# davmacario/MDI-LLM

Measured on AMD Instinct MI355X. Metric: llama3_8b_pipeline_decode_tok_per_s, higher is better.
Workload: dtype bf16; 1 GPU; model=Meta-Llama-3-8B-Instruct, global_batch=1, seq_len=128, max_seq_len=2048, parallelism=pp1, samples_in_flight=1, group_size=1, backend=hip

## Files before the change

mdi_llm_amd/ops/hip/decode_kernels.hip:

```cpp

#include <cstdlib>
#include <type_traits>
#include <hip/hip_runtime.h>
#include <hip/hip_bf16.h>

#include "decode_kernels.h"

#define DEVINL __device__ __forceinline__

using bf16 = __hip_bfloat16;

DEVINL float b2f(bf16 v) { return __bfloat162float(v); }
DEVINL bf16 f2b(float v) { return __float2bfloat16(v); }

struct bf16x8 {
  bf16 v[8];
};

DEVINL bf16x8 load8(const bf16* p) {
  bf16x8 r;
  *reinterpret_cast<int4*>(r.v) = *reinterpret_cast<const int4*>(p);
  return r;
}

using i32x4_t = __attribute__((ext_vector_type(4))) int;

DEVINL bf16x8 load8_nt(const bf16* p) {
  bf16x8 r;
  *reinterpret_cast<i32x4_t*>(r.v) =
      __builtin_nontemporal_load(reinterpret_cast<const i32x4_t*>(p));
  return r;
}

DEVINL i32x4_t load16_nt_u8(const unsigned char* p) {
  return __builtin_nontemporal_load(reinterpret_cast<const i32x4_t*>(p));
}

using f32x4 = __attribute__((__vector_size__(16))) float;
using bf16x8_t = __attribute__((ext_vector_type(8))) __bf16;

DEVINL float wave_reduce_max(float v) {
#pragma unroll
  for (int off = 32; off > 0; off >>= 1)
    v = fmaxf(v, __shfl_xor(v, off, 64));
  return v;
}

using u8kv = unsigned char;
typedef float v2fkv __attribute__((ext_vector_type(2)));

DEVINL u8kv f32_to_fp8(float f) {
  const int packed = __builtin_amdgcn_cvt_pk_fp8_f32(f, 0.f, 0, false);
  return (u8kv)(packed & 0xFF);
}

DEVINL float fp8_to_f32(u8kv v) {
  return __builtin_amdgcn_cvt_f32_fp8((int)v, 0);
}

DEVINL bf16x8_t fp8x8_to_bf16(const u8kv* p, float scl) {
  const int lo = *reinterpret_cast<const int*>(p);
  const int hi = *reinterpret_cast<const int*>(p + 4);
  const v2fkv a = __builtin_amdgcn_cvt_pk_f32_fp8(lo, false);
  const v2fkv b = __builtin_amdgcn_cvt_pk_f32_fp8(lo, true);
  const v2fkv c = __builtin_amdgcn_cvt_pk_f32_fp8(hi, false);
  const v2fkv d = __builtin_amdgcn_cvt_pk_f32_fp8(hi, true);
  bf16x8_t r;
  r[0] = (__bf16)(a.x * scl);
  r[1] = (__bf16)(a.y * scl);
  r[2] = (__bf16)(b.x * scl);
  r[3] = (__bf16)(b.y * scl);
  r[4] = (__bf16)(c.x * scl);
  r[5] = (__bf16)(c.y * scl);
  r[6] = (__bf16)(d.x * scl);
  r[7] = (__bf16)(d.y * scl);
  return r;
}

DEVINL void fp8x8_fma(float* o, float pw, const u8kv* p, float scl) {
  const int lo = *reinterpret_cast<const int*>(p);
  const int hi = *reinterpret_cast<const int*>(p + 4);
  const v2fkv a = __builtin_amdgcn_cvt_pk_f32_fp8(lo, false);
  const v2fkv b = __builtin_amdgcn_cvt_pk_f32_fp8(lo, true);
  const v2fkv c = __builtin_amdgcn_cvt_pk_f32_fp8(hi, false);
  const v2fkv d = __builtin_amdgcn_cvt_pk_f32_fp8(hi, true);
  const float ps = pw * scl;
  o[0] += ps * a.x;
  o[1] += ps * a.y;
  o[2] += ps * b.x;
  o[3] += ps * b.y;
  o[4] += ps * c.x;
  o[5] += ps * c.y;
  o[6] += ps * d.x;
  o[7] += ps * d.y;
}

DEVINL void lds_fmax_u(unsigned* addr, float v) {
  atomicMax(addr, __float_as_uint(v));
}

DEVINL float wave_reduce_sum(float v) {
#pragma unroll
  for (int off = 32; off > 0; off >>= 1) v += __shfl_xor(v, off, 64);
  return v;
}

__global__ void rmsnorm_kernel(bf16* __restrict__ out,
                               const bf16* __restrict__ x,
                               const bf16* __restrict__ w, int n, float eps) {
  __shared__ float red[4];
  out += (size_t)blockIdx.y * n;
  x += (size_t)blockIdx.y * n;
  const int tid = threadIdx.x;
  float acc = 0.f;
  for (int i = tid * 8; i < n; i += blockDim.x * 8) {
    bf16x8 v = load8(x + i);
#pragma unroll
    for (int j = 0; j < 8; ++j) {
      float f = b2f(v.v[j]);
      acc += f * f;
    }
  }
  acc = wave_reduce_sum(acc);
  if ((tid & 63) == 0) red[tid >> 6] = acc;
  __syncthreads();
  float total = red[0] + red[1] + red[2] + red[3];
  float scale = rsqrtf(total / n + eps);
  for (int i = tid * 8; i < n; i += blockDim.x * 8) {
    bf16x8 v = load8(x + i);
    bf16x8 g = load8(w + i);
    bf16x8 o;
#pragma unroll
    for (int j = 0; j < 8; ++j)
      o.v[j] = f2b(b2f(v.v[j]) * scale * b2f(g.v[j]));
    *reinterpret_cast<int4*>(out + i) = *reinterpret_cast<const int4*>(o.v);
  }
}

__global__ void layernorm_kernel(bf16* __restrict__ out,
                                 const bf16* __restrict__ x,
                                 const bf16* __restrict__ w,
                                 const bf16* __restrict__ b, int n,
                                 float eps) {
  __shared__ float red[8];
  const int tid = threadIdx.x;
  float s = 0.f, s2 = 0.f;
  for (int i = tid * 8; i < n; i += blockDim.x * 8) {
    bf16x8 v = load8(x + i);
#pragma unroll
    for (int j = 0; j < 8; ++j) {
      float f = b2f(v.v[j]);
      s += f;
      s2 += f * f;
    }
  }
  s = wave_reduce_sum(s);
  s2 = wave_reduce_sum(s2);
  if ((tid & 63) == 0) {
    red[(tid >> 6) * 2] = s;
    red[(tid >> 6) * 2 + 1] = s2;
  }
  __syncthreads();
  float mean = (red[0] + red[2] + red[4] + red[6]) / n;
  float var = (red[1] + red[3] + red[5] + red[7]) / n - mean * mean;
  float inv = rsqrtf(var + eps);
  for (int i = tid * 8; i < n; i += blockDim.x * 8) {
    bf16x8 v = load8(x + i);
    bf16x8 g = load8(w + i);
    bf16x8 o;
    if (b != nullptr) {
      bf16x8 bb = load8(b + i);
#pragma unroll
      for (int j = 0; j < 8; ++j)
        o.v[j] = f2b((b2f(v.v[j]) - mean) * inv * b2f(g.v[j]) + b2f(bb.v[j]));
    } else {
#pragma unroll
      for (int j = 0; j < 8; ++j)
// ... 865 lines not shown
  }
}

__global__ void swiglu_mul_kernel(bf16* __restrict__ out,
                                  const bf16* __restrict__ g,
                                  const bf16* __restrict__ u,
                                  long long n, int gelu_gate) {
  const long long i0 = ((long long)blockIdx.x * blockDim.x + threadIdx.x) * 8;
  const long long stride = (long long)gridDim.x * blockDim.x * 8;
  for (long long i = i0; i < n; i += stride) {
    bf16x8 gv = load8(g + i);
    bf16x8 uv = load8(u + i);
    bf16x8 o;
#pragma unroll
    for (int j = 0; j < 8; ++j) {
      const float gf = b2f(gv.v[j]);
      const float act = gelu_gate ? gelu_tanh(gf)
                                  : gf / (1.f + __expf(-gf));
      o.v[j] = f2b(act * b2f(uv.v[j]));
    }
    *reinterpret_cast<int4*>(out + i) = *reinterpret_cast<const int4*>(o.v);
  }
}

__global__ void embed_kernel(bf16* __restrict__ out,
                             const bf16* __restrict__ wte,
                             const int* __restrict__ token, int n_embd,
                             float scale) {
  const int t = token[0];
  const bf16* row = wte + (size_t)t * n_embd;
  for (int i = (blockIdx.x * blockDim.x + threadIdx.x) * 8; i < n_embd;
       i += gridDim.x * blockDim.x * 8) {
    bf16x8 v = load8(row + i);
    if (scale != 1.f) {
#pragma unroll
      for (int j = 0; j < 8; ++j) v.v[j] = f2b(b2f(v.v[j]) * scale);
    }
    *reinterpret_cast<int4*>(out + i) = *reinterpret_cast<const int4*>(v.v);
  }
}

__global__ void rope_kv_append_kernel(
    bf16* __restrict__ qkv, bf16* __restrict__ kpool,
    bf16* __restrict__ vpool, const float* __restrict__ cos_t,
    const float* __restrict__ sin_t, const int* __restrict__ pos_p,
    const int* __restrict__ slot_p, int layer, int n_layers_pool,
    int n_kv_heads, int max_seq, int head_size, int rope_n_elem, int qpk) {
  const int g = blockIdx.x;
  const int pos = pos_p[0];
  const int slot = slot_p[0];
  const int tid = threadIdx.x;
  const int half = rope_n_elem >> 1;

  bf16* base = qkv + (size_t)g * (qpk + 2) * head_size;

  for (int idx = tid; idx < (qpk + 1) * half; idx += blockDim.x) {
    const int r = idx / half;
    const int d = idx % half;
    bf16* row = base + (size_t)r * head_size;
    float x1 = b2f(row[d]);
    float x2 = b2f(row[d + half]);
    float c1 = cos_t[(size_t)pos * rope_n_elem + d];
    float s1 = sin_t[(size_t)pos * rope_n_elem + d];
    float c2 = cos_t[(size_t)pos * rope_n_elem + d + half];
    float s2 = sin_t[(size_t)pos * rope_n_elem + d + half];
    row[d] = f2b(x1 * c1 - x2 * s1);
    row[d + half] = f2b(x2 * c2 + x1 * s2);
  }
  __syncthreads();

  const size_t cache_off =
      (((size_t)slot * n_layers_pool + layer) * n_kv_heads + g) *
          (size_t)max_seq * head_size +
      (size_t)pos * head_size;
  const bf16* krow = base + (size_t)qpk * head_size;
  const bf16* vrow = base + (size_t)(qpk + 1) * head_size;
  for (int d = tid; d < head_size; d += blockDim.x) {
    kpool[cache_off + d] = krow[d];
    vpool[cache_off + d] = vrow[d];
  }
}

#define ATTN_WAVES 4
#define ATTN_BLOCK_MAX_SEQ 4096

template <int HS>
DEVINL int q_swz(int row, int d) {
  int byte = (row * HS + d) * 2;
  byte ^= (row & 7) << 4;
  return byte >> 1;
}

DEVINL float rope_elem(const bf16* row, int d, int ne,
                       const float* __restrict__ cos_t,
                       const float* __restrict__ sin_t, int pos) {
  float x = b2f(row[d]);
  if (d >= ne) return x;
  const int half = ne >> 1;
  const float c = cos_t[(size_t)pos * ne + d];
  const float s = sin_t[(size_t)pos * ne + d];
  if (d < half) return x * c - b2f(row[d + half]) * s;
  return x * c + b2f(row[d - half]) * s;
}

template <int QPK, int HS, int BATCH, int KV8>
__global__ void attn_decode_block_kernel(
    bf16* __restrict__ out,
    const bf16* __restrict__ qkv,
    void* __restrict__ kpool_v, void* __restrict__ vpool_v,
    float* __restrict__ kscale, float* __restrict__ vscale,
    const float* __restrict__ cos_t, const float* __restrict__ sin_t,
    int rope_ne, const int* __restrict__ pos_p,
    const int* __restrict__ slot_p, int layer, int n_layers_pool,
    int n_kv_heads, int max_seq, float scale, int n_batch) {
  using kvt = std::conditional_t<KV8 != 0, u8kv, bf16>;
  kvt* kpool = reinterpret_cast<kvt*>(kpool_v);
  kvt* vpool = reinterpret_cast<kvt*>(vpool_v);
  constexpr int head_size = HS;
  static_assert(HS % 32 == 0 && HS * QPK >= 64, "unsupported attn geometry");
  constexpr int ODIM = HS * QPK / 64;

  __shared__ __attribute__((aligned(16))) bf16 q_lds[16 * HS];
  __shared__ __attribute__((aligned(16))) bf16 k_cur[HS];
  __shared__ float o_part[ATTN_WAVES][QPK][HS];
  __shared__ float ml_part[ATTN_WAVES][QPK][2];
  __shared__ unsigned kvmax[2];

  const int wave = threadIdx.x >> 6;
  const int lane = threadIdx.x & 63;
  const int b = BATCH ? (int)blockIdx.x / n_kv_heads : 0;
  const int g = BATCH ? (int)blockIdx.x % n_kv_heads : (int)blockIdx.x;
  if (b >= n_batch) return;

  const int S = pos_p[b] + 1;
  const int pos = S - 1;
  const int slot = slot_p[b];
  const int n_head_all = n_kv_heads * QPK;
  if (BATCH) {
    const int qkv_dim = n_kv_heads * (QPK + 2) * head_size;
    qkv += (size_t)b * qkv_dim;
    out += (size_t)b * n_head_all * head_size;
  }

  const size_t cache_base =
      (((size_t)slot * n_layers_pool + layer) * n_kv_heads + g) *
      (size_t)max_seq * head_size;
  const size_t scl_base =
      (((size_t)slot * n_layers_pool + layer) * n_kv_heads + g) *
      (size_t)max_seq;
  const bf16* krow_cur = qkv + ((size_t)g * (QPK + 2) + QPK) * head_size;
  const bf16* vrow_cur = krow_cur + head_size;
  if (KV8 && threadIdx.x < 2) kvmax[threadIdx.x] = 0;

  for (int i = threadIdx.x; i < (16 - QPK) * head_size / 8; i += 256)
    reinterpret_cast<bf16x8_t*>(q_lds + QPK * head_size)[i] = bf16x8_t{};
  for (int i = threadIdx.x; i < QPK * head_size; i += 256) {
    const int r = i / head_size;
    const int d = i % head_size;
    const bf16* qrow = qkv + ((size_t)g * (QPK + 2) + r) * head_size;
    q_lds[q_swz<HS>(r, d)] =
        f2b(rope_elem(qrow, d, rope_ne, cos_t, sin_t, pos));
  }
  for (int d = threadIdx.x; d < head_size; d += 256)
    k_cur[d] = f2b(rope_elem(krow_cur, d, rope_ne, cos_t, sin_t, pos));
  __syncthreads();

  if constexpr (KV8) {
    float lk = 0.f, lv = 0.f;
    for (int d = threadIdx.x; d < head_size; d += 256) {
      lk = fmaxf(lk, fabsf(b2f(k_cur[d])));
      lv = fmaxf(lv, fabsf(b2f(vrow_cur[d])));
    }
    lds_fmax_u(&kvmax[0], lk);
    lds_fmax_u(&kvmax[1], lv);
    __syncthreads();
    const float ks = fmaxf(__uint_as_float(kvmax[0]), 1e-12f) / 448.f;
    const float vs = fmaxf(__uint_as_float(kvmax[1]), 1e-12f) / 448.f;
    for (int d = threadIdx.x; d < head_size; d += 256) {
      kpool[cache_base + (size_t)pos * head_size + d] =
          f32_to_fp8(b2f(k_cur[d]) / ks);
      vpool[cache_base + (size_t)pos * head_size + d] =
          f32_to_fp8(b2f(vrow_cur[d]) / vs);
    }
    if (threadIdx.x == 0) {
      kscale[scl_base + pos] = ks;
      vscale[scl_base + pos] = vs;
    }
  } else {
    for (int d = threadIdx.x; d < head_size; d += 256) {
      kpool[cache_base + (size_t)pos * head_size + d] = k_cur[d];
      vpool[cache_base + (size_t)pos * head_size + d] = vrow_cur[d];
    }
  }

  const int qa = lane & 15;
  const int sub = lane >> 4;
  const int qb = lane % QPK;
  const int d0 = (lane / QPK) * ODIM;

  float m_st = -1e30f, l_st = 0.f;
  float o_acc[ODIM];
#pragma unroll
  for (int i = 0; i < ODIM; ++i) o_acc[i] = 0.f;

  const int n_tiles = (S + 15) / 16;
  for (int t = wave; t < n_tiles; t += ATTN_WAVES) {
    const int key0 = t * 16;

    f32x4 acc4 = {0.f, 0.f, 0.f, 0.f};
    const int arow = lane & 15;
    const int koff = (lane >> 4) * 8;
    const int akey = key0 + arow;
    const kvt* krow = kpool + cache_base + (size_t)akey * head_size;
    const bool row_valid = akey < S;
    const bool row_cur = akey == pos;
    float kscl = 1.f;
    if (KV8 && row_valid && !row_cur) kscl = kscale[scl_base + akey];
#pragma unroll
    for (int c = 0; c < HS / 32; ++c) {
      bf16x8_t af = {};
      if (row_cur)
        af = *reinterpret_cast<const bf16x8_t*>(&k_cur[c * 32 + koff]);
      else if (row_valid) {
        if constexpr (KV8)
          af = fp8x8_to_bf16(
              reinterpret_cast<const u8kv*>(krow) + c * 32 + koff, kscl);
        else
          af = *reinterpret_cast<const bf16x8_t*>(
              reinterpret_cast<const bf16*>(krow) + c * 32 + koff);
      }
      const bf16x8_t bq = *reinterpret_cast<const bf16x8_t*>(
          &q_lds[q_swz<HS>(arow, c * 32 + koff)]);
      acc4 = __builtin_amdgcn_mfma_f32_16x16x32_bf16(af, bq, acc4, 0, 0, 0);
    }
    float sc[4];
#pragma unroll
    for (int r = 0; r < 4; ++r) {
      const int key = key0 + sub * 4 + r;
      sc[r] = (key < S) ? acc4[r] * scale : -1e30f;
    }

    float tmax = fmaxf(fmaxf(sc[0], sc[1]), fmaxf(sc[2], sc[3]));
    tmax = fmaxf(tmax, __shfl_xor(tmax, 16, 64));
    tmax = fmaxf(tmax, __shfl_xor(tmax, 32, 64));
    const float m_new = fmaxf(m_st, tmax);
    const float alpha = __expf(m_st - m_new);
    m_st = m_new;
    float e[4];
    float psum = 0.f;
#pragma unroll
    for (int r = 0; r < 4; ++r) {
      const int key = key0 + sub * 4 + r;
      e[r] = (key < S) ? __expf(sc[r] - m_new) : 0.f;
      psum += e[r];
    }
    psum += __shfl_xor(psum, 16, 64);
    psum += __shfl_xor(psum, 32, 64);
    l_st = l_st * alpha + psum;

    const float alphaB = __shfl(alpha, qb, 64);
#pragma unroll
    for (int i = 0; i < ODIM; ++i) o_acc[i] *= alphaB;
#pragma unroll
    for (int s = 0; s < 16; ++s) {
      const float p = __shfl(e[s & 3], ((s >> 2) << 4) | qb, 64);
      const int skey = min(key0 + s, pos);
      const bool vcur = skey == pos;
      const bf16* vrow_b = vrow_cur + d0;
      const kvt* vrow_p = vpool + cache_base + (size_t)skey * head_size + d0;
      float vscl = 1.f;
      if (KV8 && !vcur) vscl = vscale[scl_base + skey];
      if constexpr (ODIM >= 8) {
#pragma unroll
        for (int i = 0; i < ODIM; i += 8) {
          if (!vcur) {
            if constexpr (KV8) {
              fp8x8_fma(&o_acc[i], p,
                        reinterpret_cast<const u8kv*>(vrow_p) + i, vscl);
              continue;
            }
          }
          bf16x8_t vv;
          if (vcur) {
            vv = *reinterpret_cast<const bf16x8_t*>(vrow_b + i);
          } else {
            vv = *reinterpret_cast<const bf16x8_t*>(
                reinterpret_cast<const bf16*>(vrow_p) + i);
          }
#pragma unroll
          for (int j = 0; j < 8; ++j) o_acc[i + j] += p * (float)vv[j];
        }
      } else {
#pragma unroll
        for (int j = 0; j < ODIM; ++j) {
          float v;
          if (vcur)
            v = b2f(vrow_b[j]);
          else if constexpr (KV8)
            v = fp8_to_f32(reinterpret_cast<const u8kv*>(vrow_p)[j]) * vscl;
          else
            v = b2f(reinterpret_cast<const bf16*>(vrow_p)[j]);
          o_acc[j] += p * v;
        }
      }
    }
  }

#pragma unroll
  for (int i = 0; i < ODIM; ++i) o_part[wave][qb][d0 + i] = o_acc[i];
  if (lane < QPK) {
    ml_part[wave][lane][0] = m_st;
    ml_part[wave][lane][1] = l_st;
  }
  __syncthreads();

  for (int i = threadIdx.x; i < QPK * head_size; i += 256) {
    const int h = i / head_size;
    const int d = i % head_size;
    float M = -1e30f;
#pragma unroll
    for (int w = 0; w < ATTN_WAVES; ++w)
      M = fmaxf(M, ml_part[w][h][0]);
    float den = 0.f, num = 0.f;
#pragma unroll
    for (int w = 0; w < ATTN_WAVES; ++w) {
      const float wgt = __expf(ml_part[w][h][0] - M);
      den += wgt * ml_part[w][h][1];
      num += wgt * o_part[w][h][d];
    }
    out[(size_t)(g * QPK + h) * head_size + d] = f2b(num / den);
  }
}

typedef __attribute__((address_space(1))) unsigned int gu32_t;

template <int QPK, int HS, int THROTTLE>
__global__ void attn_proj_kernel(
    bf16* __restrict__ out,
    const bf16* __restrict__ qkv,
    bf16* __restrict__ kpool, bf16* __restrict__ vpool,
    const float* __restrict__ cos_t, const float* __restrict__ sin_t,
    int rope_ne, const int* __restrict__ pos_p,
    const int* __restrict__ slot_p, int layer, int n_layers_pool,
    int n_kv_heads, int max_seq, float scale,
    const bf16* __restrict__ W,
    const bf16* __restrict__ bias,
    const bf16* __restrict__ res,
    unsigned int* __restrict__ gran,
    int M, int BR) {
  constexpr int head_size = HS;
  constexpr int ODIM = HS * QPK / 64;
  extern __shared__ __attribute__((aligned(16))) char smem[];

  const int K = n_kv_heads * QPK * head_size;
  const int tid = threadIdx.x;
  const int wave = tid >> 6;
  const int lane = tid & 63;
  const int S = pos_p[0] + 1;
  const int pos = S - 1;
  const int slot = slot_p[0];
  const unsigned tag = (unsigned)(slot * max_seq + S);
  gu32_t* g32 = (gu32_t*)gran;
  gu32_t* flags = g32 + K / 2;

  if ((int)blockIdx.x >= n_kv_heads) {
    const int pb = (int)blockIdx.x - n_kv_heads;
    const int PBe = (int)gridDim.x - n_kv_heads;
    bf16* wlds = reinterpret_cast<bf16*>(smem);
    int* vflag = reinterpret_cast<int*>(smem + (size_t)BR * K * 2);
    volatile int* yready = vflag + 1;
    const bf16* ygl = reinterpret_cast<const bf16*>(gran);
    bool polled = false;
    bool y_ok = true;
    if (tid == 0) *yready = 0;
    __syncthreads();
    for (int row0 = pb * BR; row0 < M; row0 += PBe * BR) {
      if (row0 != pb * BR) __syncthreads();
      const int nr = min(BR, M - row0);
      {
        const int chunks = nr * (K / 8);
        int i = tid;
        for (; i + 3 * 256 < chunks; i += 4 * 256) {
          if (THROTTLE > 0 && !polled && !*yready) {
            if (lane == 0) {
              const unsigned f = __hip_atomic_load(
                  &flags[wave & (n_kv_heads - 1)], __ATOMIC_RELAXED,
                  __HIP_MEMORY_SCOPE_AGENT);
              if (f == tag) *yready = 1;
            }
            __builtin_amdgcn_s_sleep(THROTTLE);
          }
          bf16x8 w0, w1, w2, w3;
#pragma unroll
          for (int u = 0; u < 4; ++u) {
            const int ii = i + u * 256;
            const int r = ii / (K / 8);
            const int c = ii - r * (K / 8);
            bf16x8 wv = load8_nt(W + (size_t)(row0 + r) * K + c * 8);
            if (u == 0) w0 = wv;
            else if (u == 1) w1 = wv;
            else if (u == 2) w2 = wv;
            else w3 = wv;
          }
#pragma unroll
          for (int u = 0; u < 4; ++u) {
            const int ii = i + u * 256;
            const int r = ii / (K / 8);
            const int c = ii - r * (K / 8);
// ... 1689 lines not shown
  switch (norm_kind) {
    case 1: SW4_CASE(1); break;
    case 2: SW4_CASE(2); break;
    default: SW4_CASE(0);
  }
#undef SW4_CASE
}

void launch_gemv_swiglu(void* out, const void* Wg, const void* Wu,
                        const void* x, const void* norm_w, const void* norm_b,
                        float eps, int M, int K, int gelu_gate, int norm_kind,
                        const int* eidx, long long estride,
                        const float* escale, hipStream_t stream) {
  const int smem = K * sizeof(bf16);
  dim3 grid(gemv_grid(M, 4)), block(256);
#define SW_CASE(N)                                                          \
  hipLaunchKernelGGL((gemv_swiglu_kernel<N>), grid, block, smem, stream,    \
                     (bf16*)out, (const bf16*)Wg, (const bf16*)Wu,          \
                     (const bf16*)x, (const bf16*)norm_w,                   \
                     (const bf16*)norm_b, eps, M, K, gelu_gate, eidx,       \
                     estride, escale)
  switch (norm_kind) {
    case 1: SW_CASE(1); break;
    case 2: SW_CASE(2); break;
    default: SW_CASE(0);
  }
#undef SW_CASE
}

void launch_swiglu_mul(void* out, const void* g, const void* u,
                       long long n, int gelu_gate, hipStream_t stream) {
  long long blocks = (n / 8 + 255) / 256;
  if (blocks > 4096) blocks = 4096;
  if (blocks < 1) blocks = 1;
  hipLaunchKernelGGL(swiglu_mul_kernel, dim3((unsigned)blocks), dim3(256),
                     0, stream, (bf16*)out, (const bf16*)g, (const bf16*)u,
                     n, gelu_gate);
}

void launch_moe_gate_topk(int* eidx, float* escale, const void* logits,
                          int n_e, int k, hipStream_t stream) {
  hipLaunchKernelGGL(moe_gate_topk_kernel, dim3(1), dim3(64), 0, stream,
                     eidx, escale, (const bf16*)logits, n_e, k);
}

void launch_embed(void* out, const void* wte, const int* token, int n_embd,
                  float scale, hipStream_t stream) {
  int blocks = (n_embd / 8 + 255) / 256;
  hipLaunchKernelGGL(embed_kernel, dim3(blocks > 0 ? blocks : 1), dim3(256),
                     0, stream, (bf16*)out, (const bf16*)wte, token, n_embd,
                     scale);
}

void launch_rope_kv_append(void* qkv, void* kpool, void* vpool,
                           const float* cos_t, const float* sin_t,
                           const int* pos, const int* slot, int layer,
                           int n_layers_pool, int n_kv_heads, int max_seq,
                           int head_size, int rope_n_elem, int qpk,
                           hipStream_t stream) {
  hipLaunchKernelGGL(rope_kv_append_kernel, dim3(n_kv_heads), dim3(256), 0,
                     stream, (bf16*)qkv, (bf16*)kpool, (bf16*)vpool, cos_t,
                     sin_t, pos, slot, layer, n_layers_pool, n_kv_heads,
                     max_seq, head_size, rope_n_elem, qpk);
}

template <int QPK, int HS>
static void attn_dispatch2(void* out, float* part_o, float* part_ml,
                           const void* qkv, void* kpool, void* vpool,
                           float* kscale, float* vscale,
                           const float* cos_t, const float* sin_t,
                           int rope_ne, const int* pos, const int* slot,
                           int layer, int n_layers_pool, int n_kv_heads,
                           int max_seq, int n_chunks, float scale,
                           int n_batch, int blocks, int force_split,
                           hipStream_t stream) {
  const int kv8 = kscale != nullptr;
  static int force_splits = -1;
  if (force_splits < 0) {
    const char* e = getenv("MDI_ATTN_FORCE_SPLITS");
    force_splits = (e && e[0] == '1') ? 1 : 0;
  }
  if (max_seq <= ATTN_BLOCK_MAX_SEQ && !force_splits && !force_split) {
    const int nb = (n_batch > 0 ? n_batch : 1) * n_kv_heads;
#define ATTN_BLK(BATCHV, KV8V, NBATCH)                                      \
    hipLaunchKernelGGL((attn_decode_block_kernel<QPK, HS, BATCHV, KV8V>),   \
                       dim3(nb), dim3(256), 0, stream, (bf16*)out,          \
                       (const bf16*)qkv, kpool, vpool, kscale, vscale,      \
                       cos_t, sin_t, rope_ne, pos, slot, layer,             \
                       n_layers_pool, n_kv_heads, max_seq, scale, NBATCH)
    if (n_batch > 0) {
      if (kv8) ATTN_BLK(1, 1, n_batch);
      else ATTN_BLK(1, 0, n_batch);
    } else {
      if (kv8) ATTN_BLK(0, 1, 1);
      else ATTN_BLK(0, 0, 1);
    }
#undef ATTN_BLK
    return;
  }
#define ATTN_SPL(BATCHV, KV8V, NBATCH)                                      \
  hipLaunchKernelGGL((attn_decode_kernel<QPK, HS, BATCHV, KV8V>),           \
                     dim3(blocks), dim3(256), 0, stream, part_o, part_ml,   \
                     (const bf16*)qkv, kpool, vpool, kscale, vscale, cos_t, \
                     sin_t, rope_ne, pos, slot, layer, n_layers_pool,       \
                     n_kv_heads, max_seq, n_chunks, scale, NBATCH)
  if (n_batch > 0) {
    if (kv8) ATTN_SPL(1, 1, n_batch);
    else ATTN_SPL(1, 0, n_batch);
  } else {
    if (kv8) ATTN_SPL(0, 1, 1);
    else ATTN_SPL(0, 0, 1);
  }
#undef ATTN_SPL
}

template <int QPK>
static int attn_dispatch1(int head_size, void* out, float* part_o,
                          float* part_ml, const void* qkv, void* kpool,
                          void* vpool, float* kscale, float* vscale,
                          const float* cos_t,
                          const float* sin_t, int rope_ne, const int* pos,
                          const int* slot, int layer, int n_layers_pool,
                          int n_kv_heads, int max_seq, int n_chunks,
                          float scale, int n_batch, int blocks,
                          int force_split, hipStream_t stream) {
#define CASE_HS(H)                                                          \
  if (head_size == H) {                                                     \
    if constexpr (QPK * H >= 64) {                                          \
      attn_dispatch2<QPK, H>(out, part_o, part_ml, qkv, kpool, vpool,       \
                             kscale, vscale, cos_t, sin_t, rope_ne, pos,    \
                             slot, layer, n_layers_pool, n_kv_heads,        \
                             max_seq, n_chunks, scale, n_batch, blocks,     \
                             force_split, stream);                          \
      return 0;                                                             \
    }                                                                       \
  }
  CASE_HS(64)
  CASE_HS(128)
  CASE_HS(256)
#undef CASE_HS
  return -1;
}

int launch_attn_decode(void* out, float* part_o, float* part_ml,
                       const void* qkv, void* kpool, void* vpool,
                       float* kscale, float* vscale,
                       const float* cos_t, const float* sin_t, int rope_ne,
                       const int* pos, const int* slot, int layer,
                       int n_layers_pool, int n_kv_heads, int max_seq,
                       int head_size, int qpk, int n_chunks, float scale,
                       int n_batch, int force_split, hipStream_t stream) {
  const int n_wg = n_kv_heads * n_chunks * (n_batch > 0 ? n_batch : 1);
  const int blocks = (n_wg + ATTN_WAVES - 1) / ATTN_WAVES;
  int rc = -1;
  switch (qpk) {
    case 1:
      rc = attn_dispatch1<1>(
          head_size, out, part_o, part_ml, qkv, kpool, vpool, kscale,
          vscale, cos_t, sin_t,
          rope_ne, pos, slot, layer, n_layers_pool, n_kv_heads, max_seq,
          n_chunks, scale, n_batch, blocks, force_split, stream);
      break;
    case 2:
      rc = attn_dispatch1<2>(
          head_size, out, part_o, part_ml, qkv, kpool, vpool, kscale,
          vscale, cos_t, sin_t,
          rope_ne, pos, slot, layer, n_layers_pool, n_kv_heads, max_seq,
          n_chunks, scale, n_batch, blocks, force_split, stream);
      break;
    case 4:
      rc = attn_dispatch1<4>(
          head_size, out, part_o, part_ml, qkv, kpool, vpool, kscale,
          vscale, cos_t, sin_t,
          rope_ne, pos, slot, layer, n_layers_pool, n_kv_heads, max_seq,
          n_chunks, scale, n_batch, blocks, force_split, stream);
      break;
    case 8:
      rc = attn_dispatch1<8>(
// ... 128 lines not shown
```

Baseline: 289.4 tokens/s.

## Widen non-batched attention block, prefetch first KV tile, vectorize RoPE

The non-batched single-block decode attention kernel now picks its wave count at compile time from LDS and register budgets, so it can run more than the fixed ATTN_WAVES. For bf16 KV, each wave loads its first K tile (and its V rows when ODIM is 8) into registers before the RoPE and cache-write phase. This hides cache-read latency behind that setup work. RoPE for Q and the current K is vectorized to 8-element loads. The costs are higher register pressure and more code paths.

```diff
diff --git a/mdi_llm_amd/ops/hip/decode_kernels.hip b/mdi_llm_amd/ops/hip/decode_kernels.hip
--- a/mdi_llm_amd/ops/hip/decode_kernels.hip
+++ b/mdi_llm_amd/ops/hip/decode_kernels.hip
@@ -1145,8 +1145,19 @@
   return x * c + b2f(row[d - half]) * s;
 }
 
-template <int QPK, int HS, int BATCH, int KV8>
-__global__ void attn_decode_block_kernel(
+template <int QPK, int HS, int KV8>
+constexpr int attn_block_waves() {
+  constexpr int ODIM = QPK * HS / 64;
+  constexpr int w_lds =
+      16 * QPK * HS * 4 <= 65536 ? 16 : 8 * QPK * HS * 4 <= 65536 ? 8 : 4;
+  constexpr int w_reg = (ODIM <= 8 ? 16 : ODIM <= 16 ? 8 : 4) / (KV8 ? 2 : 1);
+  constexpr int w = w_lds < w_reg ? w_lds : w_reg;
+  return w < 4 ? 4 : w;
+}
+
+template <int QPK, int HS, int BATCH, int KV8, int W>
+__global__ void __launch_bounds__(BATCH ? 1024 : W * 64)
+attn_decode_block_kernel(
     bf16* __restrict__ out,
     const bf16* __restrict__ qkv,
     void* __restrict__ kpool_v, void* __restrict__ vpool_v,
@@ -1159,13 +1170,16 @@
   kvt* kpool = reinterpret_cast<kvt*>(kpool_v);
   kvt* vpool = reinterpret_cast<kvt*>(vpool_v);
   constexpr int head_size = HS;
+  constexpr int NT = W * 64;
   static_assert(HS % 32 == 0 && HS * QPK >= 64, "unsupported attn geometry");
   constexpr int ODIM = HS * QPK / 64;
+  constexpr bool EARLY_K = !KV8 && !BATCH;
+  constexpr bool EARLY_V = !KV8 && !BATCH && ODIM == 8;
 
   __shared__ __attribute__((aligned(16))) bf16 q_lds[16 * HS];
   __shared__ __attribute__((aligned(16))) bf16 k_cur[HS];
-  __shared__ float o_part[ATTN_WAVES][QPK][HS];
-  __shared__ float ml_part[ATTN_WAVES][QPK][2];
+  __shared__ float o_part[W][QPK][HS];
+  __shared__ float ml_part[W][QPK][2];
   __shared__ unsigned kvmax[2];
 
   const int wave = threadIdx.x >> 6;
@@ -1177,6 +1191,7 @@
   const int S = pos_p[b] + 1;
   const int pos = S - 1;
   const int slot = slot_p[b];
+  const int n_tiles = (S + 15) / 16;
   const int n_head_all = n_kv_heads * QPK;
   if (BATCH) {
     const int qkv_dim = n_kv_heads * (QPK + 2) * head_size;
@@ -1194,22 +1209,86 @@
   const bf16* vrow_cur = krow_cur + head_size;
   if (KV8 && threadIdx.x < 2) kvmax[threadIdx.x] = 0;
 
-  for (int i = threadIdx.x; i < (16 - QPK) * head_size / 8; i += 256)
+  const int arow = lane & 15;
+  const int koff = (lane >> 4) * 8;
+  const int sub = lane >> 4;
+  const int qb = lane % QPK;
+  const int d0 = (lane / QPK) * ODIM;
+
+  bf16x8_t k_pre[EARLY_K ? HS / 32 : 1];
+  bf16x8_t v_pre[EARLY_V ? 16 : 1];
+  if (wave < n_tiles) {
+    if constexpr (EARLY_K) {
+      const int akey = wave * 16 + arow;
+#pragma unroll
+      for (int c = 0; c < HS / 32; ++c) {
+        k_pre[c] = bf16x8_t{};
+        if (akey < pos)
+          k_pre[c] = *reinterpret_cast<const bf16x8_t*>(
+              reinterpret_cast<const bf16*>(kpool) + cache_base +
+              (size_t)akey * head_size + c * 32 + koff);
+      }
+    }
+    if constexpr (EARLY_V) {
+#pragma unroll
+      for (int s = 0; s < 16; ++s) {
+        const int skey = min(wave * 16 + s, pos);
+        const bf16* vp =
+            skey == pos ? vrow_cur + d0
+                        : reinterpret_cast<const bf16*>(vpool) + cache_base +
+                              (size_t)skey * head_size + d0;
+        v_pre[s] = *reinterpret_cast<const bf16x8_t*>(vp);
+      }
+    }
+  }
+
+  for (int i = threadIdx.x; i < (16 - QPK) * head_size / 8; i += NT)
     reinterpret_cast<bf16x8_t*>(q_lds + QPK * head_size)[i] = bf16x8_t{};
-  for (int i = threadIdx.x; i < QPK * head_size; i += 256) {
-    const int r = i / head_size;
-    const int d = i % head_size;
-    const bf16* qrow = qkv + ((size_t)g * (QPK + 2) + r) * head_size;
-    q_lds[q_swz<HS>(r, d)] =
-        f2b(rope_elem(qrow, d, rope_ne, cos_t, sin_t, pos));
-  }
-  for (int d = threadIdx.x; d < head_size; d += 256)
-    k_cur[d] = f2b(rope_elem(krow_cur, d, rope_ne, cos_t, sin_t, pos));
+  if (rope_ne > 0 && (rope_ne & 15) == 0) {
+    const int half = rope_ne >> 1;
+    for (int u = threadIdx.x; u < (QPK + 1) * (HS / 8); u += NT) {
+      const int r = u / (HS / 8);
+      const int d = (u % (HS / 8)) * 8;
+      const bf16* row = qkv + ((size_t)g * (QPK + 2) + r) * head_size;
+      bf16x8_t x = *reinterpret_cast<const bf16x8_t*>(row + d);
+      if (d < rope_ne) {
+        const bool lo = d < half;
+        const bf16x8_t pr = *reinterpret_cast<const bf16x8_t*>(
+            row + (lo ? d + half : d - half));
+        const float* cp = cos_t + (size_t)pos * rope_ne + d;
+        const float* sp = sin_t + (size_t)pos * rope_ne + d;
+        const f32x4 c0 = *reinterpret_cast<const f32x4*>(cp);
+        const f32x4 c1 = *reinterpret_cast<const f32x4*>(cp + 4);
+        const f32x4 s0 = *reinterpret_cast<const f32x4*>(sp);
+        const f32x4 s1 = *reinterpret_cast<const f32x4*>(sp + 4);
+#pragma unroll
+        for (int j = 0; j < 8; ++j) {
+          const float xf = (float)x[j];
+          const float pv = (float)pr[j];
+          const float c = j < 4 ? c0[j & 3] : c1[j & 3];
+          const float s = j < 4 ? s0[j & 3] : s1[j & 3];
+          x[j] = (__bf16)(lo ? xf * c - pv * s : xf * c + pv * s);
+        }
+      }
+      bf16* dst = r < QPK ? &q_lds[q_swz<HS>(r, d)] : &k_cur[d];
+      *reinterpret_cast<bf16x8_t*>(dst) = x;
+    }
+  } else {
+    for (int i = threadIdx.x; i < QPK * head_size; i += NT) {
+      const int r = i / head_size;
+      const int d = i % head_size;
+      const bf16* qrow = qkv + ((size_t)g * (QPK + 2) + r) * head_size;
+      q_lds[q_swz<HS>(r, d)] =
+          f2b(rope_elem(qrow, d, rope_ne, cos_t, sin_t, pos));
+    }
+    for (int d = threadIdx.x; d < head_size; d += NT)
+      k_cur[d] = f2b(rope_elem(krow_cur, d, rope_ne, cos_t, sin_t, pos));
+  }
   __syncthreads();
 
   if constexpr (KV8) {
     float lk = 0.f, lv = 0.f;
-    for (int d = threadIdx.x; d < head_size; d += 256) {
+    for (int d = threadIdx.x; d < head_size; d += NT) {
       lk = fmaxf(lk, fabsf(b2f(k_cur[d])));
       lv = fmaxf(lv, fabsf(b2f(vrow_cur[d])));
     }
@@ -1218,7 +1297,7 @@
     __syncthreads();
     const float ks = fmaxf(__uint_as_float(kvmax[0]), 1e-12f) / 448.f;
     const float vs = fmaxf(__uint_as_float(kvmax[1]), 1e-12f) / 448.f;
-    for (int d = threadIdx.x; d < head_size; d += 256) {
+    for (int d = threadIdx.x; d < head_size; d += NT) {
       kpool[cache_base + (size_t)pos * head_size + d] =
           f32_to_fp8(b2f(k_cur[d]) / ks);
       vpool[cache_base + (size_t)pos * head_size + d] =
@@ -1229,29 +1308,23 @@
       vscale[scl_base + pos] = vs;
     }
   } else {
-    for (int d = threadIdx.x; d < head_size; d += 256) {
+    for (int d = threadIdx.x; d < head_size; d += NT) {
       kpool[cache_base + (size_t)pos * head_size + d] = k_cur[d];
       vpool[cache_base + (size_t)pos * head_size + d] = vrow_cur[d];
     }
   }
 
-  const int qa = lane & 15;
-  const int sub = lane >> 4;
-  const int qb = lane % QPK;
-  const int d0 = (lane / QPK) * ODIM;
-
   float m_st = -1e30f, l_st = 0.f;
   float o_acc[ODIM];
 #pragma unroll
   for (int i = 0; i < ODIM; ++i) o_acc[i] = 0.f;
 
-  const int n_tiles = (S + 15) / 16;
-  for (int t = wave; t < n_tiles; t += ATTN_WAVES) {
+  auto do_tile = [&](const int t, auto first)
+                     __attribute__((always_inline)) {
+    constexpr bool FIRST = decltype(first)::value;
     const int key0 = t * 16;
 
     f32x4 acc4 = {0.f, 0.f, 0.f, 0.f};
-    const int arow = lane & 15;
-    const int koff = (lane >> 4) * 8;
     const int akey = key0 + arow;
     const kvt* krow = kpool + cache_base + (size_t)akey * head_size;
     const bool row_valid = akey < S;
@@ -1263,6 +1336,8 @@
       bf16x8_t af = {};
       if (row_cur)
         af = *reinterpret_cast<const bf16x8_t*>(&k_cur[c * 32 + koff]);
+      else if constexpr (FIRST && EARLY_K)
+        af = k_pre[c];
       else if (row_valid) {
         if constexpr (KV8)
           af = fp8x8_to_bf16(
@@ -1323,7 +1398,9 @@
             }
           }
           bf16x8_t vv;
-          if (vcur) {
+          if constexpr (FIRST && EARLY_V) {
+            vv = v_pre[s];
+          } else if (vcur) {
             vv = *reinterpret_cast<const bf16x8_t*>(vrow_b + i);
           } else {
             vv = *reinterpret_cast<const bf16x8_t*>(
@@ -1346,6 +1423,12 @@
         }
       }
     }
+  };
+  if constexpr (EARLY_K) {
+    if (wave < n_tiles) do_tile(wave, std::true_type{});
+    for (int t = wave + W; t < n_tiles; t += W) do_tile(t, std::false_type{});
+  } else {
+    for (int t = wave; t < n_tiles; t += W) do_tile(t, std::false_type{});
   }
 
 #pragma unroll
@@ -1356,16 +1439,16 @@
   }
   __syncthreads();
 
-  for (int i = threadIdx.x; i < QPK * head_size; i += 256) {
+  for (int i = threadIdx.x; i < QPK * head_size; i += NT) {
     const int h = i / head_size;
     const int d = i % head_size;
     float M = -1e30f;
 #pragma unroll
-    for (int w = 0; w < ATTN_WAVES; ++w)
+    for (int w = 0; w < W; ++w)
       M = fmaxf(M, ml_part[w][h][0]);
     float den = 0.f, num = 0.f;
 #pragma unroll
-    for (int w = 0; w < ATTN_WAVES; ++w) {
+    for (int w = 0; w < W; ++w) {
       const float wgt = __expf(ml_part[w][h][0] - M);
       den += wgt * ml_part[w][h][1];
       num += wgt * o_part[w][h][d];
@@ -3221,18 +3304,20 @@
   }
   if (max_seq <= ATTN_BLOCK_MAX_SEQ && !force_splits && !force_split) {
     const int nb = (n_batch > 0 ? n_batch : 1) * n_kv_heads;
-#define ATTN_BLK(BATCHV, KV8V, NBATCH)                                      \
-    hipLaunchKernelGGL((attn_decode_block_kernel<QPK, HS, BATCHV, KV8V>),   \
-                       dim3(nb), dim3(256), 0, stream, (bf16*)out,          \
-                       (const bf16*)qkv, kpool, vpool, kscale, vscale,      \
-                       cos_t, sin_t, rope_ne, pos, slot, layer,             \
-                       n_layers_pool, n_kv_heads, max_seq, scale, NBATCH)
+    constexpr int WIDE = attn_block_waves<QPK, HS, 0>();
+    constexpr int WIDE8 = attn_block_waves<QPK, HS, 1>();
+#define ATTN_BLK(BATCHV, KV8V, NBATCH, WV)                                  \
+    hipLaunchKernelGGL(                                                     \
+        (attn_decode_block_kernel<QPK, HS, BATCHV, KV8V, WV>), dim3(nb),    \
+        dim3(WV * 64), 0, stream, (bf16*)out, (const bf16*)qkv, kpool,      \
+        vpool, kscale, vscale, cos_t, sin_t, rope_ne, pos, slot, layer,     \
+        n_layers_pool, n_kv_heads, max_seq, scale, NBATCH)
     if (n_batch > 0) {
-      if (kv8) ATTN_BLK(1, 1, n_batch);
-      else ATTN_BLK(1, 0, n_batch);
+      if (kv8) ATTN_BLK(1, 1, n_batch, ATTN_WAVES);
+      else ATTN_BLK(1, 0, n_batch, ATTN_WAVES);
     } else {
-      if (kv8) ATTN_BLK(0, 1, 1);
-      else ATTN_BLK(0, 0, 1);
+      if (kv8) ATTN_BLK(0, 1, 1, WIDE8);
+      else ATTN_BLK(0, 0, 1, WIDE);
     }
 #undef ATTN_BLK
     return;
```

Result: no change. 289.6 tokens/s (median of 3 runs) (+0.1%).

## Prefetch KV tiles into registers and widen single-batch attention block waves

Applied to the files above, without the earlier changes.

The block decode attention kernel now issues K and V cache loads for its first tile before the Q RoPE/LDS setup, and groups V-row loads into register batches ahead of the FMAs, so global-memory latency overlaps with other work. The wave count becomes a template parameter, and the non-batched bf16 path launches up to 16 waves per KV head, giving more parallelism over the sequence. The current-token KV cache write (including the FP8 scale computation) is moved after the main loop, and reads for the current key are served from LDS or registers. This raises register pressure and the shared memory used for per-wave partials.

```diff
diff --git a/mdi_llm_amd/ops/hip/decode_kernels.hip b/mdi_llm_amd/ops/hip/decode_kernels.hip
--- a/mdi_llm_amd/ops/hip/decode_kernels.hip
+++ b/mdi_llm_amd/ops/hip/decode_kernels.hip
@@ -58,9 +58,7 @@
   return __builtin_amdgcn_cvt_f32_fp8((int)v, 0);
 }
 
-DEVINL bf16x8_t fp8x8_to_bf16(const u8kv* p, float scl) {
-  const int lo = *reinterpret_cast<const int*>(p);
-  const int hi = *reinterpret_cast<const int*>(p + 4);
+DEVINL bf16x8_t fp8x8_to_bf16(int lo, int hi, float scl) {
   const v2fkv a = __builtin_amdgcn_cvt_pk_f32_fp8(lo, false);
   const v2fkv b = __builtin_amdgcn_cvt_pk_f32_fp8(lo, true);
   const v2fkv c = __builtin_amdgcn_cvt_pk_f32_fp8(hi, false);
@@ -77,9 +75,12 @@
   return r;
 }
 
-DEVINL void fp8x8_fma(float* o, float pw, const u8kv* p, float scl) {
-  const int lo = *reinterpret_cast<const int*>(p);
-  const int hi = *reinterpret_cast<const int*>(p + 4);
+DEVINL bf16x8_t fp8x8_to_bf16(const u8kv* p, float scl) {
+  return fp8x8_to_bf16(*reinterpret_cast<const int*>(p),
+                       *reinterpret_cast<const int*>(p + 4), scl);
+}
+
+DEVINL void fp8x8_fma(float* o, float pw, int lo, int hi, float scl) {
   const v2fkv a = __builtin_amdgcn_cvt_pk_f32_fp8(lo, false);
   const v2fkv b = __builtin_amdgcn_cvt_pk_f32_fp8(lo, true);
   const v2fkv c = __builtin_amdgcn_cvt_pk_f32_fp8(hi, false);
@@ -93,6 +94,11 @@
   o[5] += ps * c.y;
   o[6] += ps * d.x;
   o[7] += ps * d.y;
+}
+
+DEVINL void fp8x8_fma(float* o, float pw, const u8kv* p, float scl) {
+  fp8x8_fma(o, pw, *reinterpret_cast<const int*>(p),
+            *reinterpret_cast<const int*>(p + 4), scl);
 }
 
 DEVINL void lds_fmax_u(unsigned* addr, float v) {
@@ -1124,6 +1130,7 @@
 }
 
 #define ATTN_WAVES 4
+#define ATTN_BLOCK_WAVES_B1 16
 #define ATTN_BLOCK_MAX_SEQ 4096
 
 template <int HS>
@@ -1145,8 +1152,77 @@
   return x * c + b2f(row[d - half]) * s;
 }
 
-template <int QPK, int HS, int BATCH, int KV8>
-__global__ void attn_decode_block_kernel(
+template <int QPK, int HS>
+constexpr int attn_block_waves(int want) {
+  int nw = want;
+  while (nw > 4 && nw * QPK * HS * 4 > 32768) nw >>= 1;
+  return nw;
+}
+
+using i32x2_t = __attribute__((ext_vector_type(2))) int;
+template <int KV8>
+struct kv_raw8 {
+  using type = bf16x8_t;
+};
+template <>
+struct kv_raw8<1> {
+  using type = i32x2_t;
+};
+
+template <int ODIM, int KV8>
+struct VFrag {
+  static constexpr int NV = ODIM >= 8 ? ODIM / 8 : 1;
+  static constexpr int NE = ODIM >= 8 ? 1 : ODIM;
+  static constexpr int REGS = ODIM >= 8 ? NV * (KV8 ? 2 : 4) : ODIM;
+  using raw8 = typename kv_raw8<KV8>::type;
+  using elt = std::conditional_t<KV8 != 0, u8kv, bf16>;
+  raw8 r8[NV];
+  elt e[NE];
+  float scl;
+};
+
+template <int ODIM, int KV8>
+DEVINL void vfrag_load(VFrag<ODIM, KV8>& f,
+                       const typename VFrag<ODIM, KV8>::elt* row) {
+  using VF = VFrag<ODIM, KV8>;
+  if constexpr (ODIM >= 8) {
+#pragma unroll
+    for (int i = 0; i < VF::NV; ++i)
+      f.r8[i] = *reinterpret_cast<const typename VF::raw8*>(row + i * 8);
+  } else {
+#pragma unroll
+    for (int j = 0; j < ODIM; ++j) f.e[j] = row[j];
+  }
+}
+
+template <int ODIM, int KV8>
+DEVINL void vfrag_fma(float* o, float p, const VFrag<ODIM, KV8>& f) {
+  using VF = VFrag<ODIM, KV8>;
+  if constexpr (ODIM >= 8) {
+#pragma unroll
+    for (int i = 0; i < VF::NV; ++i) {
+      if constexpr (KV8) {
+        fp8x8_fma(o + i * 8, p, f.r8[i][0], f.r8[i][1], f.scl);
+      } else {
+#pragma unroll
+        for (int j = 0; j < 8; ++j) o[i * 8 + j] += p * (float)f.r8[i][j];
+      }
+    }
+  } else {
+#pragma unroll
+    for (int j = 0; j < ODIM; ++j) {
+      float v;
+      if constexpr (KV8)
+        v = fp8_to_f32(f.e[j]) * f.scl;
+      else
+        v = b2f(f.e[j]);
+      o[j] += p * v;
+    }
+  }
+}
+
+template <int QPK, int HS, int BATCH, int KV8, int NW>
+__global__ __launch_bounds__(NW * 64) void attn_decode_block_kernel(
     bf16* __restrict__ out,
     const bf16* __restrict__ qkv,
     void* __restrict__ kpool_v, void* __restrict__ vpool_v,
@@ -1161,14 +1237,23 @@
   constexpr int head_size = HS;
   static_assert(HS % 32 == 0 && HS * QPK >= 64, "unsupported attn geometry");
   constexpr int ODIM = HS * QPK / 64;
+  constexpr int NT = NW * 64;
+  constexpr int KC = HS / 32;
+  using raw8 = typename kv_raw8<KV8>::type;
+  using VF = VFrag<ODIM, KV8>;
+  constexpr int VBUDGET = (BATCH || NW >= 16) ? 16 : 128;
+  constexpr int VPF = VBUDGET / VF::REGS < 1
+                          ? 1
+                          : (VBUDGET / VF::REGS > 16 ? 16
+                                                     : VBUDGET / VF::REGS);
 
   __shared__ __attribute__((aligned(16))) bf16 q_lds[16 * HS];
   __shared__ __attribute__((aligned(16))) bf16 k_cur[HS];
-  __shared__ float o_part[ATTN_WAVES][QPK][HS];
-  __shared__ float ml_part[ATTN_WAVES][QPK][2];
+  __shared__ float o_part[NW][QPK][HS];
+  __shared__ float ml_part[NW][QPK][2];
   __shared__ unsigned kvmax[2];
 
-  const int wave = threadIdx.x >> 6;
+  const int wave = __builtin_amdgcn_readfirstlane(threadIdx.x >> 6);
   const int lane = threadIdx.x & 63;
   const int b = BATCH ? (int)blockIdx.x / n_kv_heads : 0;
   const int g = BATCH ? (int)blockIdx.x % n_kv_heads : (int)blockIdx.x;
@@ -1194,82 +1279,95 @@
   const bf16* vrow_cur = krow_cur + head_size;
   if (KV8 && threadIdx.x < 2) kvmax[threadIdx.x] = 0;
 
-  for (int i = threadIdx.x; i < (16 - QPK) * head_size / 8; i += 256)
+  const int sub = lane >> 4;
+  const int qb = lane % QPK;
+  const int d0 = (lane / QPK) * ODIM;
+  const int arow = lane & 15;
+  const int koff = (lane >> 4) * 8;
+
+  const int n_tiles = (S + 15) / 16;
+  const int pmax = pos > 0 ? pos - 1 : 0;
+  raw8 kf[KC];
+  float kscl = 1.f;
+  VF vpre[VPF];
+  VFrag<ODIM, 0> vcf;
+  auto load_k = [&](int tile) __attribute__((always_inline)) {
+    const int akey = min(tile * 16 + arow, pmax);
+    const kvt* krow = kpool + cache_base + (size_t)akey * head_size + koff;
+#pragma unroll
+    for (int c = 0; c < KC; ++c)
+      kf[c] = *reinterpret_cast<const raw8*>(krow + c * 32);
+    if constexpr (KV8) kscl = kscale[scl_base + akey];
+  };
+  auto load_v = [&](VF& f, int key) __attribute__((always_inline)) {
+    const int skey = min(key, pmax);
+    vfrag_load<ODIM, KV8>(
+        f, vpool + cache_base + (size_t)skey * head_size + d0);
+    if constexpr (KV8) f.scl = vscale[scl_base + skey];
+  };
+  int t = wave;
+  if (t < n_tiles) {
+    load_k(t);
+#pragma unroll
+    for (int s = 0; s < VPF; ++s) load_v(vpre[s], t * 16 + s);
+    vfrag_load<ODIM, 0>(vcf, vrow_cur + d0);
+  }
+
+  for (int i = threadIdx.x; i < (16 - QPK) * head_size / 8; i += NT)
     reinterpret_cast<bf16x8_t*>(q_lds + QPK * head_size)[i] = bf16x8_t{};
-  for (int i = threadIdx.x; i < QPK * head_size; i += 256) {
+  for (int i = threadIdx.x; i < QPK * head_size; i += NT) {
     const int r = i / head_size;
     const int d = i % head_size;
     const bf16* qrow = qkv + ((size_t)g * (QPK + 2) + r) * head_size;
     q_lds[q_swz<HS>(r, d)] =
         f2b(rope_elem(qrow, d, rope_ne, cos_t, sin_t, pos));
   }
-  for (int d = threadIdx.x; d < head_size; d += 256)
+  for (int d = threadIdx.x; d < head_size; d += NT)
     k_cur[d] = f2b(rope_elem(krow_cur, d, rope_ne, cos_t, sin_t, pos));
   __syncthreads();
 
-  if constexpr (KV8) {
-    float lk = 0.f, lv = 0.f;
-    for (int d = threadIdx.x; d < head_size; d += 256) {
-      lk = fmaxf(lk, fabsf(b2f(k_cur[d])));
-      lv = fmaxf(lv, fabsf(b2f(vrow_cur[d])));
-    }
-    lds_fmax_u(&kvmax[0], lk);
-    lds_fmax_u(&kvmax[1], lv);
-    __syncthreads();
-    const float ks = fmaxf(__uint_as_float(kvmax[0]), 1e-12f) / 448.f;
-    const float vs = fmaxf(__uint_as_float(kvmax[1]), 1e-12f) / 448.f;
-    for (int d = threadIdx.x; d < head_size; d += 256) {
-      kpool[cache_base + (size_t)pos * head_size + d] =
-          f32_to_fp8(b2f(k_cur[d]) / ks);
-      vpool[cache_base + (size_t)pos * head_size + d] =
-          f32_to_fp8(b2f(vrow_cur[d]) / vs);
-    }
-    if (threadIdx.x == 0) {
-      kscale[scl_base + pos] = ks;
-      vscale[scl_base + pos] = vs;
-    }
-  } else {
-    for (int d = threadIdx.x; d < head_size; d += 256) {
-      kpool[cache_base + (size_t)pos * head_size + d] = k_cur[d];
-      vpool[cache_base + (size_t)pos * head_size + d] = vrow_cur[d];
-    }
-  }
-
-  const int qa = lane & 15;
-  const int sub = lane >> 4;
-  const int qb = lane % QPK;
-  const int d0 = (lane / QPK) * ODIM;
+  const int ad = NT - 1 - (int)threadIdx.x;
+  if (ad < head_size) {
+    if constexpr (KV8) {
+      lds_fmax_u(&kvmax[0], fabsf(b2f(k_cur[ad])));
+      lds_fmax_u(&kvmax[1], fabsf(b2f(vrow_cur[ad])));
+    } else {
+      kpool[cache_base + (size_t)pos * head_size + ad] = k_cur[ad];
+      vpool[cache_base + (size_t)pos * head_size + ad] = vrow_cur[ad];
+    }
+  }
 
   float m_st = -1e30f, l_st = 0.f;
   float o_acc[ODIM];
 #pragma unroll
   for (int i = 0; i < ODIM; ++i) o_acc[i] = 0.f;
 
-  const int n_tiles = (S + 15) / 16;
-  for (int t = wave; t < n_tiles; t += ATTN_WAVES) {
+  for (; t < n_tiles; t += NW) {
     const int key0 = t * 16;
+    if (t != wave) {
+      load_k(t);
+#pragma unroll
+      for (int s = 0; s < VPF; ++s) load_v(vpre[s], key0 + s);
+    }
 
     f32x4 acc4 = {0.f, 0.f, 0.f, 0.f};
-    const int arow = lane & 15;
-    const int koff = (lane >> 4) * 8;
     const int akey = key0 + arow;
-    const kvt* krow = kpool + cache_base + (size_t)akey * head_size;
-    const bool row_valid = akey < S;
+    const bool row_cached = akey < pos;
     const bool row_cur = akey == pos;
-    float kscl = 1.f;
-    if (KV8 && row_valid && !row_cur) kscl = kscale[scl_base + akey];
-#pragma unroll
-    for (int c = 0; c < HS / 32; ++c) {
+    const bool tile_cur = (pos >> 4) == t;
+#pragma unroll
+    for (int c = 0; c < KC; ++c) {
       bf16x8_t af = {};
-      if (row_cur)
-        af = *reinterpret_cast<const bf16x8_t*>(&k_cur[c * 32 + koff]);
-      else if (row_valid) {
+      if (row_cached) {
         if constexpr (KV8)
-          af = fp8x8_to_bf16(
-              reinterpret_cast<const u8kv*>(krow) + c * 32 + koff, kscl);
+          af = fp8x8_to_bf16(kf[c][0], kf[c][1], kscl);
         else
-          af = *reinterpret_cast<const bf16x8_t*>(
-              reinterpret_cast<const bf16*>(krow) + c * 32 + koff);
+          af = kf[c];
+      }
+      if (tile_cur) {
+        const bf16x8_t kc =
+            *reinterpret_cast<const bf16x8_t*>(&k_cur[c * 32 + koff]);
+        if (row_cur) af = kc;
       }
       const bf16x8_t bq = *reinterpret_cast<const bf16x8_t*>(
           &q_lds[q_swz<HS>(arow, c * 32 + koff)]);
@@ -1303,48 +1401,22 @@
     const float alphaB = __shfl(alpha, qb, 64);
 #pragma unroll
     for (int i = 0; i < ODIM; ++i) o_acc[i] *= alphaB;
-#pragma unroll
-    for (int s = 0; s < 16; ++s) {
+    auto pv_row = [&](int s, const VF& f) __attribute__((always_inline)) {
       const float p = __shfl(e[s & 3], ((s >> 2) << 4) | qb, 64);
-      const int skey = min(key0 + s, pos);
-      const bool vcur = skey == pos;
-      const bf16* vrow_b = vrow_cur + d0;
-      const kvt* vrow_p = vpool + cache_base + (size_t)skey * head_size + d0;
-      float vscl = 1.f;
-      if (KV8 && !vcur) vscl = vscale[scl_base + skey];
-      if constexpr (ODIM >= 8) {
-#pragma unroll
-        for (int i = 0; i < ODIM; i += 8) {
-          if (!vcur) {
-            if constexpr (KV8) {
-              fp8x8_fma(&o_acc[i], p,
-                        reinterpret_cast<const u8kv*>(vrow_p) + i, vscl);
-              continue;
-            }
-          }
-          bf16x8_t vv;
-          if (vcur) {
-            vv = *reinterpret_cast<const bf16x8_t*>(vrow_b + i);
-          } else {
-            vv = *reinterpret_cast<const bf16x8_t*>(
-                reinterpret_cast<const bf16*>(vrow_p) + i);
-          }
-#pragma unroll
-          for (int j = 0; j < 8; ++j) o_acc[i + j] += p * (float)vv[j];
-        }
-      } else {
-#pragma unroll
-        for (int j = 0; j < ODIM; ++j) {
-          float v;
-          if (vcur)
-            v = b2f(vrow_b[j]);
-          else if constexpr (KV8)
-            v = fp8_to_f32(reinterpret_cast<const u8kv*>(vrow_p)[j]) * vscl;
-          else
-            v = b2f(reinterpret_cast<const bf16*>(vrow_p)[j]);
-          o_acc[j] += p * v;
-        }
-      }
+      if (key0 + s >= pos)
+        vfrag_fma<ODIM, 0>(o_acc, p, vcf);
+      else
+        vfrag_fma<ODIM, KV8>(o_acc, p, f);
+    };
+#pragma unroll
+    for (int s = 0; s < VPF; ++s) pv_row(s, vpre[s]);
+#pragma unroll
+    for (int s0 = VPF; s0 < 16; s0 += VPF) {
+      VF vgrp[VPF];
+#pragma unroll
+      for (int s = 0; s < VPF; ++s) load_v(vgrp[s], key0 + s0 + s);
+#pragma unroll
+      for (int s = 0; s < VPF; ++s) pv_row(s0 + s, vgrp[s]);
     }
   }
 
@@ -1356,16 +1428,31 @@
   }
   __syncthreads();
 
-  for (int i = threadIdx.x; i < QPK * head_size; i += 256) {
+  if constexpr (KV8) {
+    if (ad < head_size) {
+      const float ks = fmaxf(__uint_as_float(kvmax[0]), 1e-12f) / 448.f;
+      const float vs = fmaxf(__uint_as_float(kvmax[1]), 1e-12f) / 448.f;
+      kpool[cache_base + (size_t)pos * head_size + ad] =
+          f32_to_fp8(b2f(k_cur[ad]) / ks);
+      vpool[cache_base + (size_t)pos * head_size + ad] =
+          f32_to_fp8(b2f(vrow_cur[ad]) / vs);
+      if (ad == 0) {
+        kscale[scl_base + pos] = ks;
+        vscale[scl_base + pos] = vs;
+      }
+    }
+  }
+
+  for (int i = threadIdx.x; i < QPK * head_size; i += NT) {
     const int h = i / head_size;
     const int d = i % head_size;
     float M = -1e30f;
 #pragma unroll
-    for (int w = 0; w < ATTN_WAVES; ++w)
+    for (int w = 0; w < NW; ++w)
       M = fmaxf(M, ml_part[w][h][0]);
     float den = 0.f, num = 0.f;
 #pragma unroll
-    for (int w = 0; w < ATTN_WAVES; ++w) {
+    for (int w = 0; w < NW; ++w) {
       const float wgt = __expf(ml_part[w][h][0] - M);
       den += wgt * ml_part[w][h][1];
       num += wgt * o_part[w][h][d];
@@ -3221,18 +3308,20 @@
   }
   if (max_seq <= ATTN_BLOCK_MAX_SEQ && !force_splits && !force_split) {
     const int nb = (n_batch > 0 ? n_batch : 1) * n_kv_heads;
-#define ATTN_BLK(BATCHV, KV8V, NBATCH)                                      \
-    hipLaunchKernelGGL((attn_decode_block_kernel<QPK, HS, BATCHV, KV8V>),   \
-                       dim3(nb), dim3(256), 0, stream, (bf16*)out,          \
-                       (const bf16*)qkv, kpool, vpool, kscale, vscale,      \
-                       cos_t, sin_t, rope_ne, pos, slot, layer,             \
-                       n_layers_pool, n_kv_heads, max_seq, scale, NBATCH)
+    constexpr int NW1 = attn_block_waves<QPK, HS>(ATTN_BLOCK_WAVES_B1);
+    constexpr int NWB = ATTN_WAVES;
+#define ATTN_BLK(BATCHV, KV8V, NWV, NBATCH)                                 \
+    hipLaunchKernelGGL(                                                     \
+        (attn_decode_block_kernel<QPK, HS, BATCHV, KV8V, NWV>), dim3(nb),   \
+        dim3(NWV * 64), 0, stream, (bf16*)out, (const bf16*)qkv, kpool,     \
+        vpool, kscale, vscale, cos_t, sin_t, rope_ne, pos, slot, layer,     \
+        n_layers_pool, n_kv_heads, max_seq, scale, NBATCH)
     if (n_batch > 0) {
-      if (kv8) ATTN_BLK(1, 1, n_batch);
-      else ATTN_BLK(1, 0, n_batch);
+      if (kv8) ATTN_BLK(1, 1, NWB, n_batch);
+      else ATTN_BLK(1, 0, NWB, n_batch);
     } else {
-      if (kv8) ATTN_BLK(0, 1, 1);
-      else ATTN_BLK(0, 0, 1);
+      if (kv8) ATTN_BLK(0, 1, NWB, 1);
+      else ATTN_BLK(0, 0, NW1, 1);
     }
 #undef ATTN_BLK
     return;
```

Result: no change. 290.0 tokens/s before, 289.5 tokens/s after (-0.2%).
